# KangWelly/Assignment-for-AAE6102_GNSS-SDR

Hardware: AMD Instinct MI355X
Metric: correlator Msamples/s (acq+track), whole job (higher is better)
Workload: dtype int8 in; acquisition: f64 correlation + f64 fine search; tracking: f64

## Files before the change

### assignment-for-aae6102_gnss-sdr_amd/csrc/acq_fft.hip

```cpp
#include "gnss_internal.h"

#pragma clang fp contract(fast)

namespace gnss {

namespace {

constexpr int kRow = 2000;
constexpr int kRowPad = 2100;
constexpr int kRowThreads = 256;
constexpr int kColThreads = 256;

template <int P> struct PrimeTab;
template <> struct PrimeTab<13> {
    static constexpr double c[13] = {1.0, 0.8854560256532099, 0.5680647467311559, 0.120536680255323, -0.35460488704253545, -0.7485107481711012, -0.970941817426052, -0.9709418174260521, -0.7485107481711013, -0.3546048870425359, 0.1205366802553232, 0.5680647467311548, 0.88545602565321};
    static constexpr double s[13] = {0.0, 0.4647231720437685, 0.8229838658936564, 0.992708874098054, 0.9350162426854148, 0.6631226582407952, 0.23931566428755768, -0.23931566428755743, -0.663122658240795, -0.9350162426854147, -0.992708874098054, -0.822983865893657, -0.4647231720437684};
};
template <> struct PrimeTab<29> {
    static constexpr double c[29] = {1.0, 0.9766205557100867, 0.907575419670957, 0.7960930657056438, 0.6473862847818277, 0.46840844069979015, 0.26752833852922075, 0.05413890858541761, -0.16178199655276473, -0.37013815533991423, -0.5611870653623823, -0.7259954919231306, -0.8568571761675893, -0.9476531711828025, -0.9941379571543596, -0.9941379571543597, -0.9476531711828025, -0.8568571761675892, -0.7259954919231311, -0.5611870653623825, -0.37013815533991445, -0.16178199655276476, 0.0541389085854167, 0.2675283385292201, 0.4684084406997903, 0.6473862847818279, 0.796093065705644, 0.9075754196709569, 0.9766205557100867};
    static constexpr double s[29] = {0.0, 0.21497044021102407, 0.4198891015602646, 0.6051742151937652, 0.7621620551276365, 0.8835120444460229, 0.963549992519223, 0.9985334138511238, 0.9868265225415261, 0.9289767198167915, 0.8276889981568906, 0.6876994588534235, 0.5155538571770216, 0.3193015301359798, 0.10811901842394192, -0.10811901842394124, -0.31930153013597995, -0.5155538571770218, -0.6876994588534231, -0.8276889981568905, -0.9289767198167914, -0.9868265225415261, -0.9985334138511239, -0.9635499925192231, -0.8835120444460228, -0.7621620551276362, -0.6051742151937649, -0.41988910156026493, -0.21497044021102438};
};

template <class V> struct RealOf;
template <> struct RealOf<float2> { using T = float; };
// ... 1258 lines not shown

size_t acq_fused_sync_bytes() { return sizeof(FuseSync); }
size_t acq_fused_err_offset() { return offsetof(FuseSync, err); }
size_t acq_fused_ring_bytes(int64_t S) { return sizeof(double2) * (size_t)kFuseX * kFuseSlots * (size_t)S; }

hipError_t launch_acq_fft_correlate_fused(const double2* C, const double2* X, int64_t S, int datalen, int nbins,
                                          int nprn, int nslot, const double2* tw_row, const double2* tw_col,
                                          double2* ring, void* sync, double* corr, hipStream_t s)
{
    if (nslot < 2 || nslot > kFuseSlots) return hipErrorInvalidValue;
    const double scale = 1.0 / ((double)S * (double)S);
    int dev = 0, ncu = 0;
    hipError_t e = hipGetDevice(&dev);
    if (e == hipSuccess) e = hipDeviceGetAttribute(&ncu, hipDeviceAttributeMultiprocessorCount, dev);
    if (e == hipSuccess) e = hipMemsetAsync(sync, 0, sizeof(FuseSync), s);
    if (e != hipSuccess) return e;
    FuseSync* sy = static_cast<FuseSync*>(sync);
#define GNSS_FUSED(P_)                                                                          \
    if (S == (int64_t)P_ * kRow) {                                                              \
        int occ = 0;                                                                            \
        e = hipOccupancyMaxActiveBlocksPerMultiprocessor(&occ, inv_fused_kernel_f64<P_>, kRowThreads, 0); \
        if (e != hipSuccess) return e;                                                          \
        const int grid = ncu * std::min(occ, 2);                                                \
        if (grid < 1) return hipErrorInvalidConfiguration;                                      \
        hipLaunchKernelGGL(inv_fused_kernel_f64<P_>, dim3(grid), dim3(kRowThreads), 0, s, C, X, nbins, nprn, \
                           datalen, nbins * nprn, nslot, scale, tw_row, tw_col, ring, sy, corr); \
        return hipGetLastError();                                                               \
    }
    GNSS_FUSED(13) GNSS_FUSED(29)
#undef GNSS_FUSED
    return hipErrorInvalidValue;
}

bool fine_fft_supported(int64_t S, int L) { return acq_fft_supported(S) && L == kFineT; }

namespace {
struct FineLayout {
    int64_t M, N, tabs, slab, part;
};
FineLayout fine_layout(int64_t S, int L, int datalen)
{
    FineLayout f;
    f.M = (int64_t)L * S;
    f.N = f.M * datalen;
    f.tabs = kRow + (int64_t)kRow * datalen + (int64_t)kFineT * kRow + S + f.M / kRow + kTwIK;
    f.slab = f.N;
    f.part = (int64_t)datalen * (kRow / kFineJC);
    return f;
}
}

static size_t fine_prep_offset(const FineLayout& f, int nsv)
{
    const size_t b = sizeof(double2) * (size_t)(f.tabs + (int64_t)nsv * f.slab) + sizeof(FineBest) * (size_t)(nsv * f.part);
    return (b + 255) & ~(size_t)255;
}
size_t fine_fft_scratch_bytes(int64_t S, int L, int datalen, int nsv)
{
    const FineLayout f = fine_layout(S, L, datalen);
    if (!GNSS_FINE_PREP) return fine_prep_offset(f, nsv);
    return fine_prep_offset(f, nsv) + (size_t)nsv * f.M * (sizeof(double2) + sizeof(float));
}

hipError_t launch_fine_fft_tables(int64_t S, int L, int datalen, void* scratch, hipStream_t s)
{
    const int64_t M = (int64_t)L * S;
    double2* tw_row = static_cast<double2*>(scratch);
    double2* tabA = tw_row + kRow;
    double2* tabB = tabA + (int64_t)kRow * datalen;
    double2* tabK = tabB + (int64_t)kFineT * kRow;
    double2* tabS = tabK + S;
    const int64_t lens[5] = {kRow, (int64_t)kRow * datalen, (int64_t)kFineT * kRow, S, M / kRow};
    const int64_t divs[5] = {kRow, (int64_t)kRow * datalen, (int64_t)kFineT * kRow, M, M / kRow};
    const int64_t rows[5] = {0, kRow, kRow, kRow, 0};
    double2* tabs[5] = {tw_row, tabA, tabB, tabK, tabS};
    for (int t = 0; t < 5; t++)
        hipLaunchKernelGGL(fine_twiddle_kernel, dim3((unsigned)((lens[t] + 255) / 256)), dim3(256), 0,
                           s, tabs[t], lens[t], divs[t], rows[t]);
    hipLaunchKernelGGL(fine_twik_kernel, dim3((kTwIK + 255) / 256), dim3(256), 0, s, tw_row, tabS + M / kRow);
    return hipGetLastError();
}

hipError_t launch_fine_fft_argmax(const int8_t* iq, const double2* xs, int64_t S, int L, int datalen,
                                  const int32_t* cd, int nsv, const float* ca, double Fs, double codeFreqBasis,
                                  double codelength, int shifted, void* scratch, int64_t* kbest, hipStream_t s)
{
    if (nsv < 1 || nsv > 65535) return hipErrorInvalidValue;
    const FineLayout f = fine_layout(S, L, datalen);
    const int64_t N = f.N;
    double2* tw_row = static_cast<double2*>(scratch);
    double2* tabA = tw_row + kRow;
    double2* tabB = tabA + (int64_t)kRow * datalen;
    double2* tabK = tabB + (int64_t)kFineT * kRow;
    double2* tabS = tabK + S;
    double2* E = tw_row + f.tabs;
    FineBest* part = reinterpret_cast<FineBest*>(E + (int64_t)nsv * f.slab);
    char* prep = static_cast<char*>(scratch) + fine_prep_offset(f, nsv);
    float* ct = reinterpret_cast<float*>(prep + (size_t)nsv * f.M * sizeof(double2));
    const int nblk = kRow / kFineJC;
    auto rows = [&](auto src, auto* xt, auto kern, auto prep_kern, int tm) {
        using SrcT = decltype(src);
        if (GNSS_FINE_PREP) {
            hipLaunchKernelGGL(prep_kern, dim3((kRow + tm - 1) / tm, nsv), dim3(kRowThreads), 0, s, src, cd, S, 1 / Fs,
                               1 / codeFreqBasis, codelength, ca, xt, ct);
            src = SrcElem<SrcT>::wrap(xt);
        }
        hipLaunchKernelGGL(kern, dim3((unsigned)(f.M / kRow), datalen, nsv), dim3(kRowThreads), 0, s, src, ct, cd, S,
                           ca, 1 / Fs, 1 / codeFreqBasis, codelength, datalen, N, tw_row, tabS + f.M / kRow, tabA,
                           tabB, E);
    };
#define GNSS_FINE(P_)                                                                           \
    if (S == (int64_t)P_ * kRow) {                                                              \
        if (xs)                                                                                 \
            rows(SrcC64{xs}, reinterpret_cast<double2*>(prep), fine_rows_kernel<P_, SrcC64>,    \
                 fine_prep_kernel<P_, SrcC64>, SrcElem<SrcC64>::kTM);                           \
        else                                                                                    \
            rows(SrcIQ8{iq}, reinterpret_cast<char2*>(prep), fine_rows_kernel<P_, SrcIQ8>,      \
                 fine_prep_kernel<P_, SrcIQ8>, SrcElem<SrcIQ8>::kTM);                           \
        hipLaunchKernelGGL(fine_cols_kernel<P_>, dim3(nblk, datalen, nsv), dim3(kColThreads), 0, s, E, \
                           datalen, N, shifted, tabK, tabS, part);                                    \
        hipLaunchKernelGGL(fine_best_final_kernel, dim3(nsv), dim3(256), 0, s, part, nblk * datalen, \
                           kbest);                                                              \
        return hipGetLastError();                                                               \
    }
    GNSS_FINE(13) GNSS_FINE(29)
#undef GNSS_FINE
    return hipErrorInvalidValue;
}

}
```

### assignment-for-aae6102_gnss-sdr_amd/csrc/api_acq.cpp

```cpp
#include <cmath>
#include <cstring>
#include <vector>

#include "host.h"

using namespace gnss;
using namespace gnss::host;

namespace {
constexpr int kAcqPipeDefault = 2;
#ifndef GNSS_ACQ_FWD_SPLIT
#define GNSS_ACQ_FWD_SPLIT 1
#endif
constexpr bool kAcqFwdSplit = GNSS_ACQ_FWD_SPLIT;
constexpr int kAcqPairFront = 60;
constexpr int kFineBatch = 16;

template <class V> struct CplxReal;
template <> struct CplxReal<float2> { using T = float; };
template <> struct CplxReal<double2> { using T = double; };

template <class V>
int acq_search(gnss_ctx* ctx, const int8_t* blk, const double2* xa, int64_t S, int dl, int nb, int np,
               const gnss_signal* sg, const gnss_acq* acq, const float* ca, typename CplxReal<V>::T* corr,
// ... 300 lines not shown
        return fail(ctx, GNSS_EDEVICE, "fused correlator: a pipeline wait timed out (grid not resident)");
    ctx->timing.acq_hypothesis_samples = (int64_t)np * nb * dl * S;

    std::vector<int> acq_idx;
    for (int i = 0; i < np; i++) {
        if (diag) {
            int k = diag->n++;
            diag->prn[k] = prns[i];
            diag->SNR[k] = ph[i].snr;
            diag->fbin[k] = ph[i].fbin + 1;
            diag->codePhase[k] = ph[i].cp + 1;
            diag->peak[k] = ph[i].peak;
            diag->peak2[k] = ph[i].peak2;
        }
        if (ph[i].snr >= 12) {
            int k = out->n++;
            out->sv[k] = prns[i];
            out->SNR[k] = ph[i].snr;
            out->Doppler[k] = acq->freqMin + acq->freqStep * (double)ph[i].fbin;
            out->codedelay[k] = ph[i].cp;
            acq_idx.push_back(i);
        }
    }
    if (out->n == 0) {
        HIP_TRY(hipEventRecord(e_all.b, ctx->stream));
        HIP_TRY(hipEventSynchronize(e_all.b));
        ctx->timing.acq_ms = e_all.ms();
        ctx->timing.acq_corr_ms = ctx->timing.acq_ms;
        return fail(ctx, GNSS_ENODATA, "No satellites acquired");
    }

    if (flen < off + S * bps * (L + 1)) return fail(ctx, GNSS_EIO, "IF record too short for fine search");
    const int fshift = dtyp == 2 ? 1 : 2;
    const int na = out->n;
    const int64_t N = (int64_t)L * S * dl;
    if (N % 2) return fail(ctx, GNSS_EINDEX, "odd fftlength: MATLAB indexes past the end (:116)");
    std::vector<float> caf((size_t)na * 1023);
    std::vector<int32_t> cdh((size_t)na);
    for (int k = 0; k < na; k++) {
        generate_ca(out->sv[k], &caf[(size_t)k * 1023]);
        cdh[k] = out->codedelay[k];
    }
    DevBuf fca, fcd, fx, kb;
    HIP_TRY(fca.alloc(ctx, "acq.fca", caf.size() * sizeof(float)));
    HIP_TRY(fcd.alloc(ctx, "acq.fcd", cdh.size() * sizeof(int32_t)));
    HIP_TRY(kb.alloc(ctx, "acq.kb", sizeof(int64_t) * (size_t)na));
    HIP_TRY(hipMemcpyAsync(fca.p, caf.data(), caf.size() * sizeof(float), hipMemcpyHostToDevice, ctx->stream));
    HIP_TRY(hipMemcpyAsync(fcd.p, cdh.data(), cdh.size() * sizeof(int32_t), hipMemcpyHostToDevice, ctx->stream));
    const bool own_fine = fine_fft_supported(S, L) && !ctx->opt[GNSS_OPT_FINE_ROCFFT];
    Events e_fine;
    if (own_fine) {
        const int fb = std::min(na, kFineBatch);
        HIP_TRY(fx.alloc(ctx, "acq.fx", fine_fft_scratch_bytes(S, L, dl, fb)));
        HIP_TRY(hipEventRecord(e_fine.a, ctx->stream));
        HIP_TRY(launch_fine_fft_tables(S, L, dl, fx.p, ctx->stream));
        for (int k0 = 0; k0 < na; k0 += fb) {
            const int nk = std::min(fb, na - k0);
            HIP_TRY(launch_fine_fft_argmax(blk, xf, S, L, dl, fcd.as<int32_t>() + k0, nk,
                                           fca.as<float>() + (size_t)k0 * 1023, sg->Fs, sg->codeFreqBasis,
                                           sg->codelength, fshift, fx.p, kb.as<int64_t>() + k0, ctx->stream));
        }
    } else {
        HIP_TRY(fx.alloc(ctx, "acq.fx", sizeof(double2) * (size_t)na * N));
        rocfft_plan pl;
        if ((st = get_plan(ctx, N, na, 1, 0, &pl))) return st;
        HIP_TRY(hipEventRecord(e_fine.a, ctx->stream));
        HIP_TRY(launch_fine_build(blk, xf, S, L, fcd.as<int32_t>(), fca.as<float>(), na, sg->Fs, sg->codeFreqBasis,
                                  sg->codelength, N, fx.as<double2>(), ctx->stream));
        if ((st = run_fft(ctx, fx.p, N, na, 1, 0))) return st;
        DevBuf fscr;
        HIP_TRY(fscr.alloc(ctx, "acq.fscr", acq_scratch_bytes(1, na)));
        HIP_TRY(launch_fine_argmax(fx.as<double2>(), na, N, fshift, fscr.p, kb.as<int64_t>(), ctx->stream));
    }
    HIP_TRY(hipEventRecord(e_fine.b, ctx->stream));
    HIP_TRY(hipEventRecord(e_all.b, ctx->stream));
    std::vector<int64_t> kh((size_t)na);
    HIP_TRY(hipMemcpyAsync(kh.data(), kb.p, sizeof(int64_t) * (size_t)na, hipMemcpyDeviceToHost, ctx->stream));
    HIP_TRY(hipStreamSynchronize(ctx->stream));
    for (int k = 0; k < na; k++) {
        const double K = (double)kh[k];
        out->fineFreq[k] = (file->dataType == 2) ? (-K * (sg->Fs / (double)N) + sg->Fs / 2) : (K * (sg->Fs / (double)N));
    }
    {
        float f = 0;
        (void)hipEventElapsedTime(&f, e_all.a, e_corr.b);
        ctx->timing.acq_corr_ms = f;
    }
    ctx->timing.acq_fine_ms = e_fine.ms();
    ctx->timing.acq_ms = e_all.ms() + (iq8 ? 0.0 : e_conv.ms());
    return GNSS_OK;
}

}
```

### assignment-for-aae6102_gnss-sdr_amd/csrc/gnss_internal.h

```cpp
#pragma once

#include <hip/hip_runtime.h>
#include <stdint.h>

#include "../../include/gnss_mi355x.h"

#define GNSS_HD __host__ __device__ __forceinline__

namespace gnss {

struct Colon {
    double a, d, c;
    int64_t n;
};

GNSS_HD Colon colon_make(double a, double d, double b)
{
    Colon r{a, d, b, -1};
    if (!(a - a == 0) || !(d - d == 0) || !(b - b == 0)) return r;
    if (d == 0 || (a < b && d < 0) || (b < a && d > 0)) return r;
    double tol = 2.0 * 2.220446049250313e-16 * fmax(fabs(a), fabs(b));
    double sig = d > 0 ? 1.0 : -1.0;
    double n;
    if (a == floor(a) && d == 1) {
// ... 362 lines not shown
    int32_t cp;
    double snr;
    double peak2;
};

hipError_t launch_acq_wipe(const int8_t* iq, const double2* xs, int64_t S, int datalen, int nbins, double IF,
                           double freqMin, double freqStep, double Fs, float2* out, hipStream_t s);
hipError_t launch_acq_code(const float* ca, const int32_t* prn_slot, int nprn, int64_t S,
                           double codeFreqBasis, double Fs, float2* out, hipStream_t s);
hipError_t launch_acq_mul(const float2* code_spec, const float2* sig_spec, int nprn, int nsig,
                          int64_t S, float2* out, hipStream_t s);
hipError_t launch_acq_power(const float2* y, int nprn, int nbins, int datalen, int64_t S,
                            int first_ms, float* corr, hipStream_t s);
hipError_t launch_acq_wipe(const int8_t* iq, const double2* xs, int64_t S, int datalen, int nbins, double IF,
                           double freqMin, double freqStep, double Fs, double2* out, hipStream_t s);
hipError_t launch_acq_code(const float* ca, const int32_t* prn_slot, int nprn, int64_t S,
                           double codeFreqBasis, double Fs, double2* out, hipStream_t s);
hipError_t launch_acq_mul(const double2* code_spec, const double2* sig_spec, int nprn, int nsig,
                          int64_t S, double2* out, hipStream_t s);
hipError_t launch_acq_power(const double2* y, int nprn, int nbins, int datalen, int64_t S,
                            int first_ms, double* corr, hipStream_t s);
hipError_t launch_acq_peak(const float* corr, int nprn, int nbins, int64_t S, int cshift,
                           int perm, AcqPeak* out, void* scratch, hipStream_t s);
hipError_t launch_acq_peak(const double* corr, int nprn, int nbins, int64_t S, int cshift,
                           int perm, AcqPeak* out, void* scratch, hipStream_t s);

bool acq_fft_supported(int64_t S);
template <class V>
hipError_t launch_acq_fft_forward(const int8_t* iq, const double2* xs, int64_t S, int datalen, int nbins, double IF,
                                  double freqMin, double freqStep, double Fs, const float* ca,
                                  int nprn, double codeFreqBasis, const V* tw_row,
                                  const V* tw_col, V* B, V* X, hipStream_t s, int bin0 = 0, int nbc = -1,
                                  bool codes = true);
constexpr int kAcqCols = 1, kAcqRows = 2;
hipError_t launch_acq_fft_correlate(const float2* C, const float2* X, int64_t S, int datalen,
                                    int nbins, int nprn, int first_pair, int npair,
                                    const float2* tw_row, const float2* tw_col, float2* A,
                                    float* corr, hipStream_t s, int parts = kAcqCols | kAcqRows);
hipError_t launch_acq_fft_correlate(const double2* C, const double2* X, int64_t S, int datalen,
                                    int nbins, int nprn, int first_pair, int npair,
                                    const double2* tw_row, const double2* tw_col, double2* A,
                                    double* corr, hipStream_t s, int parts = kAcqCols | kAcqRows);
hipError_t launch_acq_fft_pair(const double2* C, const double2* X, int64_t S, int datalen, int nbins, int nprn,
                               int cols_first, int cols_n, double2* Acols, int rows_first, int rows_n,
                               const double2* Arows, const double2* tw_row, const double2* tw_col, double* corr,
                               int front, hipStream_t s);
size_t acq_fused_sync_bytes();
size_t acq_fused_err_offset();
size_t acq_fused_ring_bytes(int64_t S);
hipError_t launch_acq_fft_correlate_fused(const double2* C, const double2* X, int64_t S, int datalen, int nbins,
                                          int nprn, int nslot, const double2* tw_row, const double2* tw_col,
                                          double2* ring, void* sync, double* corr, hipStream_t s);
bool fine_fft_supported(int64_t S, int L);
size_t fine_fft_scratch_bytes(int64_t S, int L, int datalen, int nsv);
hipError_t launch_fine_fft_tables(int64_t S, int L, int datalen, void* scratch, hipStream_t s);
hipError_t launch_fine_fft_argmax(const int8_t* iq, const double2* xs, int64_t S, int L, int datalen,
                                  const int32_t* cd, int nsv, const float* ca, double Fs, double codeFreqBasis,
                                  double codelength, int shifted, void* scratch, int64_t* kbest, hipStream_t s);
hipError_t launch_fine_build(const int8_t* iq, const double2* xs, int64_t S, int L, const int32_t* codedelay,
                             const float* ca, int nsv, double Fs, double codeFreqBasis,
                             double codelength, int64_t N, double2* out, hipStream_t s);
hipError_t launch_fine_argmax(const double2* F, int nsv, int64_t N, int shifted, void* scratch,
                              int64_t* kbest, hipStream_t s);

size_t acq_scratch_bytes(int nprn, int nsv);

hipError_t launch_stage_cpx(const int8_t* src, int prec, int type, int64_t nsamp, double2* out,
                            unsigned long long* sums, hipStream_t s);
hipError_t launch_real8_to_iq8(const int8_t* src, int64_t n, int8_t* dst, hipStream_t s);
size_t prefix16_scratch_bytes(int64_t ngroups);
hipError_t launch_prefix16(const short* src, int64_t ngroups, long long* pref_i, long long* pref_q,
                           void* scratch, size_t scratch_bytes, hipStream_t s);

struct SrcIQ8 {
    const int8_t* p;
    __device__ __forceinline__ double2 at(int64_t n) const
    {
        const char2 r = *reinterpret_cast<const char2*>(p + 2 * n);
        return make_double2((double)r.x, (double)r.y);
    }
};
struct SrcC64 {
    const double2* p;
    __device__ __forceinline__ double2 at(int64_t n) const { return p[n]; }
};


GNSS_HD double cn0_moment(const double* Z, double T)
{
    double mean = 0;
    for (int k = 0; k < 20; k++) mean += Z[k];
    mean = mean / 20;
    double var = 0;
    for (int k = 0; k < 20; k++) var += (Z[k] - mean) * (Z[k] - mean);
    var = var / 19;
    const double m2v = mean * mean - var;
    const double scale = 1 / T;
    if (m2v >= 0) {
        const double NA2 = sqrt(m2v);
        const double varIQ = 0.5 * (mean - NA2);
        return fabs(10 * log10(scale * NA2 / (2 * varIQ)));
    }
    const double y = sqrt(-m2v);
    const double nr = 0, ni = scale * y;
    const double dr = 2 * (0.5 * mean), di = 2 * (0.5 * -y);
    const double den = dr * dr + di * di;
    const double zr = (nr * dr + ni * di) / den, zi = (ni * dr - nr * di) / den;
    const double lr = 10 * (log(hypot(zr, zi)) / log(10.0));
    const double li = 10 * (atan2(zi, zr) / log(10.0));
    return hypot(lr, li);
}
// ... 227 lines not shown
```

### assignment-for-aae6102_gnss-sdr_amd/csrc/host.h

```cpp
#pragma once

#include <hip/hip_runtime.h>
#include <rocfft/rocfft.h>

#include <algorithm>
#include <cstdint>
#include <cstdlib>
#include <map>
#include <string>
#include <thread>
#include <tuple>
#include <utility>
#include <vector>

#include "gnss_internal.h"
#include "group.h"

struct gnss_ctx {
    int device = 0;
    hipStream_t stream = nullptr;
    hipStream_t stream2 = nullptr;
    hipEvent_t ev_cols[2] = {}, ev_rows[2] = {};
    std::string err;
    gnss_timing timing{};
    int profiling = 0;
    std::map<std::tuple<size_t, size_t, int, int>, rocfft_plan> plans;
    void* fft_work = nullptr;
    size_t fft_work_size = 0;
    std::map<std::string, std::pair<void*, size_t>> pool;
    std::map<std::string, std::pair<void*, size_t>> pinned;
    int64_t acq_tw_S = 0;
    int acq_tw_dbl = -1;
    int acq_fp64 = 1;
    uint64_t window = 0;
    int64_t opt[GNSS_OPT_COUNT] = {};
    int lane_path = 0;
    std::vector<gnss_ctx*> members;
    bool member = false;
    int fail_chan = -1;
    gnss::group::ResidentCache<void*> resident;
};

namespace gnss {
struct AcfDev;
struct AcfExtPlan;
namespace host {

inline const char* probe_env(const char* name)
{
    return GNSS_PROBE_BUILD ? getenv(name) : nullptr;
}

constexpr int kVtSpan = 2000;

int fail(gnss_ctx* ctx, int code, const char* fmt, ...) __attribute__((format(printf, 3, 4)));

#define HIP_TRY(expr)                                                                         \
    do {                                                                                       \
        hipError_t e_ = (expr);                                                                \
        if (e_ != hipSuccess)                                                                  \
            return ::gnss::host::fail(ctx, GNSS_EDEVICE, "%s:%d %s: %s", __FILE__, __LINE__,   \
                                      #expr, hipGetErrorString(e_));                           \
    } while (0)

template <class T>
T* pinned_buffer(gnss_ctx* ctx, const char* key, size_t count, unsigned flags = hipHostMallocDefault)
{
    auto& e = ctx->pinned[key];
    const size_t want = std::max<size_t>(count * sizeof(T), 16);
    if (e.second < want) {
        if (e.first) (void)hipHostFree(e.first);
        e = {nullptr, 0};
        if (hipHostMalloc(&e.first, want, flags) != hipSuccess) return nullptr;
        e.second = want;
    }
    return static_cast<T*>(e.first);
}

struct DevBuf {
    void* p = nullptr;
    size_t n = 0;
    bool pooled = false;
    DevBuf() = default;
    DevBuf(const DevBuf&) = delete;
    DevBuf& operator=(const DevBuf&) = delete;
// ... 106 lines not shown
```

### assignment-for-aae6102_gnss-sdr_amd/csrc/track.hip

```cpp
#include "gnss_internal.h"

#include <cstddef>
#include <type_traits>
#include <utility>

namespace gnss {

namespace {

constexpr int kStampRow = 8 + 3 * kMaxBpc;

__device__ __forceinline__ unsigned long long* stamp_row(const TrkBuffers& b)
{
    const unsigned long long cnt = __hip_atomic_load(b.stamps + (size_t)kStampSlots * kStampRow,
                                                     __ATOMIC_RELAXED, __HIP_MEMORY_SCOPE_AGENT);
    return b.stamps + (cnt % kStampSlots) * kStampRow;
}

__device__ __forceinline__ void stamp_max(unsigned long long* row, int k, unsigned long long v)
{
    row[k] = v;
}

__device__ __forceinline__ int uni(int v) { return __builtin_amdgcn_readfirstlane(v); }
// ... 445 lines not shown
    if (Index >= c.sv1) cols = (int64_t)((uint32_t)(Index - c.sv1) / (uint32_t)p.nsv) + 1;
    return cols > nstep ? nstep : cols;
}

__device__ __forceinline__ void write_record_i(const TrkParams& p, const TrkBuffers& b, int ch, const TrkChan& c,
                             const StepOut& o, const LoopUpd& u, const double* s,
                             const int64_t* pre = nullptr, int part = 3)
{
    const double P_i = s[2 * p.iP], P_q = s[2 * p.iP + 1];
    const int64_t slot = c.slot;
    g_dbl* r = (g_dbl*)(b.rec + ((int64_t)ch * p.rec_cap + slot) * GNSS_NFIELDS);
    if (part & 1) {
        const int64_t col = c.nstep;
        g_i64* dvpre = (g_i64*)(b.dvpre + (int64_t)ch * (p.rec_cap + 1));
        const int64_t dvsum = (pre ? pre[0] : dvpre[col]) + o.delayValue;
        dvpre[col + 1] = dvsum;
        const int64_t nstep = col + 1;
        const int64_t cols = record_cols(p, c, o.phaseC);
        const double codedelay =
            (double)c.codedelay0 + (double)(cols == nstep ? dvsum : (pre ? pre[1] : dvpre[cols]));
        if (slot < p.rec_cap) {
            r[GNSS_F_P_i] = P_i;                     r[GNSS_F_P_q] = P_q;
            r[GNSS_F_E_i] = s[2 * p.iE];             r[GNSS_F_E_q] = s[2 * p.iE + 1];
            r[GNSS_F_L_i] = s[2 * p.iL];             r[GNSS_F_L_q] = s[2 * p.iL + 1];
            r[GNSS_F_codedelay] = codedelay;
        }
    }
    if (part & 2) {
        const int64_t pos = c.pos + p.bps * o.n;
        const double absS = (double)pos;
        const double m = fmod_pos(absS / p.dataBytesPerSample, p.Fs * p.ms);
        if (slot < p.rec_cap) {
            r[GNSS_F_PLLdiscri] = u.PLLdiscri;       r[GNSS_F_DLLdiscri] = u.DLLdiscri;
            r[GNSS_F_remChip] = o.remChip;
            r[GNSS_F_codeFreq] = u.codeFreq;         r[GNSS_F_carrierFreq] = u.carrierFreq;
            r[GNSS_F_remPhase] = o.remPhase;         r[GNSS_F_remSample] = p.conv ? m : o.remSample;
            r[GNSS_F_numSample] = (double)o.n;       r[GNSS_F_delayValue] = (double)o.delayValue;
            r[GNSS_F_absoluteSample] = absS;         r[GNSS_F_codedelay2] = m;
        }
        if (!o.phaseC && slot < b.n1) ((g_dbl*)b.p_i_1ms)[(int64_t)ch * b.n1 + slot] = P_i;
    }
}
__device__ __noinline__ void write_record(const TrkParams& p, const TrkBuffers& b, int ch, const TrkChan& c, const StepOut& o, const LoopUpd& u, const double* s)
{
    write_record_i(p, b, ch, c, o, u, s);
}


__device__ __noinline__ double cn0_estimate(const double (&Z)[20], double T)
{
    return cn0_moment(Z, T);
}

__device__ __forceinline__ void write_state_i(const TrkParams& p, const TrkBuffers& b, int ch, TrkChan* g,
                            const TrkChan& c, const StepOut& o, const LoopUpd& u, const double* s,
                            bool io = true)
{
    const double P_i = s[2 * p.iP], P_q = s[2 * p.iP + 1];
    int index_int = c.index_int + 1;
    int snrIndex = c.snrIndex;
    const double zk = P_i * P_i + P_q * P_q;
    for (int k = 0; k < 20; k++) g->Zk[k] = k == index_int - 1 ? zk : c.Zk[k];
    if (index_int % 20 == 0 && io) {
        double Z[20];
#pragma unroll
        for (int k = 0; k < 20; k++) Z[k] = k == index_int - 1 ? zk : c.Zk[k];
        const double cn = cn0_estimate(Z, 1 * p.ms * o.pdi);
        double* cn0 = o.phaseC ? b.cn0_10 : b.cn0_1;
        if (snrIndex <= p.cn0_cap) cn0[(int64_t)ch * p.cn0_cap + snrIndex - 1] = cn;
        index_int = 0;
        snrIndex += 1;
    } else if (index_int % 20 == 0) {
        index_int = 0;
        snrIndex += 1;
    }
    g->remChip = o.remChip;
    g->remPhase = o.remPhase;
    g->remSample = o.remSample;
    g->carrier_outputLast = u.carrier_output;
    g->PLLdiscriLast = u.PLLdiscri;
    g->code_outputLast = u.code_output;
    g->DLLdiscriLast = u.DLLdiscri;
    g->codeFreq = u.codeFreq;
    g->carrierFreq = u.carrierFreq;
    g->numSample = o.n;
    g->pos = c.pos + p.bps * o.n;
    g->Index = c.Index + (o.phaseC ? 10 : 1);
    g->nstep = c.nstep + 1;
    g->slot = c.slot + 1;
    g->index_int = index_int;
    g->snrIndex = snrIndex;
}
__device__ __noinline__ void write_state(const TrkParams& p, const TrkBuffers& b, int ch, TrkChan* g, const TrkChan& c, const StepOut& o, const LoopUpd& u, const double* s, bool io)
{
    write_state_i(p, b, ch, g, c, o, u, s, io);
}

__device__ __forceinline__ void update_state_inplace(const TrkParams& p, const TrkBuffers& b, int ch,
                                                     TrkChan& c, const StepOut& o, const LoopUpd& u,
                                                     const double* s, bool io)
{
    const double P_i = s[2 * p.iP], P_q = s[2 * p.iP + 1];
    int index_int = c.index_int + 1;
    int snrIndex = c.snrIndex;
    c.Zk[index_int - 1] = P_i * P_i + P_q * P_q;
    if (index_int % 20 == 0) {
        if (io) {
            double Z[20];
#pragma unroll
            for (int k = 0; k < 20; k++) Z[k] = c.Zk[k];
            const double cn = cn0_estimate(Z, 1 * p.ms * o.pdi);
            g_dbl* cn0 = (g_dbl*)(o.phaseC ? b.cn0_10 : b.cn0_1);
            if (snrIndex <= p.cn0_cap) cn0[(int64_t)ch * p.cn0_cap + snrIndex - 1] = cn;
        }
        index_int = 0;
        snrIndex += 1;
    }
    const int64_t pos = c.pos, Index = c.Index, nstep = c.nstep, slot = c.slot;
    c.remChip = o.remChip;
    c.remPhase = o.remPhase;
    c.remSample = o.remSample;
    c.carrier_outputLast = u.carrier_output;
    c.PLLdiscriLast = u.PLLdiscri;
    c.code_outputLast = u.code_output;
    c.DLLdiscriLast = u.DLLdiscri;
    c.codeFreq = u.codeFreq;
    c.carrierFreq = u.carrierFreq;
    c.numSample = o.n;
    c.pos = pos + p.bps * o.n;
    c.Index = Index + (o.phaseC ? 10 : 1);
    c.nstep = nstep + 1;
    c.slot = slot + 1;
    c.index_int = index_int;
    c.snrIndex = snrIndex;
}


}

__device__ __forceinline__ double2 ld_rcs(const StepDesc* d, int m) { return d->rcs[m]; }
__device__ __forceinline__ double2 ld_rcs(g_desc* d, int m)
{
    typedef __attribute__((address_space(1))) const double g_cdbl;
    g_cdbl* q = (g_cdbl*)&d->rcs[m];
    return make_double2(q[0], q[1]);
}

template <int SUB> struct RegRaw {
    const int4 (&r)[SUB];
    __device__ __forceinline__ int4 get(int j) const { return r[j]; }
};
struct LdsRaw {
    const int4* p;
    __device__ __forceinline__ int4 get(int j) const { return p[j * kTrkThreads]; }
};
typedef __attribute__((address_space(3))) const char lds_cchar;
typedef __attribute__((address_space(3))) const double lds_cdbl;
typedef double dbl2v __attribute__((ext_vector_type(2)));
typedef __attribute__((address_space(3))) const dbl2v lds_cdbl2;

template <class F, int... I>
__device__ __forceinline__ void static_for_seq(F&& f, std::integer_sequence<int, I...>)
{
    (f(std::integral_constant<int, I>{}), ...);
// ... 1010 lines not shown
        while ((st = __hip_atomic_load((g_u32*)state, __ATOMIC_RELAXED, __HIP_MEMORY_SCOPE_AGENT)) == 0) {
            if (wall_clock64() - t0 > 2000000ull) atomicCAS(state, 0u, 2u);
            __builtin_amdgcn_s_sleep(2);
        }
        if (st == 2) atomicCAS(w, 0u, 2u);
        s_go = st == 1;
    }
    __syncthreads();
    return s_go != 0;
}

template <int SUB>
__device__ __forceinline__ void prefetch_raw(const int8_t* iq, int64_t g0, int64_t gmax, int4* s_raw,
                                             int tid)
{
    const int wbase = tid & ~63;
#pragma unroll
    for (int j = 0; j < SUB; j++) {
        int64_t gj = g0 + j;
        gj = gj < gmax ? gj : gmax;
        __builtin_amdgcn_global_load_lds((__attribute__((address_space(1))) void*)(iq + 16 * gj),
                                         (__attribute__((address_space(3))) void*)(s_raw + j * kTrkThreads + wbase),
                                         16, 0, 0);
    }
}

#ifndef GNSS_DEFER
#define GNSS_DEFER 0
#endif
#ifndef GNSS_WPE_TAPS
#define GNSS_WPE_TAPS 2
#endif
template <int NT, int SUB, bool DIVIDE, bool VB = false, bool REGC = false>
__global__ __launch_bounds__(kTrkThreads) __attribute__((amdgpu_waves_per_eu(NT > 3 ? GNSS_WPE_TAPS : 3, NT > 3 ? GNSS_WPE_TAPS : 3))) void track_run_kernel(const TrkParams* __restrict__ pp,
                                                               const TrkBuffers* __restrict__ bp, int bpc,
                                                               int vpb, int nsteps, unsigned tag0)
{
    const TrkParams& p = *pp;
    const TailK tk = tail_k(p);
    const TrkBuffers& b = *bp;
    constexpr int M = 8 * SUB;
    constexpr int NV = 2 * NT;
    constexpr int T = kTrkThreads;
    static_assert(M <= kLaneMax, "lane span exceeds the rotation table");
    const int vpb_ = VB ? vpb : 1;
    const int pbpc = (bpc + vpb_ - 1) / vpb_;
    const bool xl = GNSS_XCD_LOCAL == 1 && !VB && p.nch == 8;
    const bool cul = GNSS_XCD_LOCAL == 2 && !VB && p.nch == 8 && pbpc == 96;
    const int ch = xl ? (int)(blockIdx.x & 7) : cul ? (int)((blockIdx.x & 255) >> 5) : (int)(blockIdx.x / pbpc);
    const int pblk = xl ? (int)(blockIdx.x >> 3)
                    : cul ? (int)((blockIdx.x & 31) * 3 + (blockIdx.x >> 8)) : (int)(blockIdx.x - ch * pbpc);
    const int blk = pblk * vpb_;
    const int nvb = VB ? (bpc - blk < vpb_ ? bpc - blk : vpb_) : 1;
    const int tid = threadIdx.x, lane = tid & 63, wv = tid >> 6;
    const bool io = pblk == 0;

    constexpr int kSlot = REGC ? 0 : 8 * T * 2;
    constexpr int kRed = red_words<run_red_taps<NT>()>();
    constexpr int kPart = run_bpc_cap(NT) * NV;
    constexpr bool kDefer = GNSS_DEFER && NT > 3;
    constexpr bool kWave1 = GNSS_DEFER == 2 && kDefer && !VB;
    static_assert(!kWave1 || GNSS_RED == 0, "GNSS_DEFER 2 needs GNSS_RED 0");
    constexpr int kPwD = run_bpc_cap(NT) * 8 + 2 * NT;
    constexpr int kStage = 2 * (NT - 1) * T;
    constexpr int kMemW = kWave1 ? kPwD + kStage + 2 * NT * 32 : 0;
    constexpr int kMem1 = kSlot > kRed ? kSlot : kRed;
    constexpr int kMem0 = kMem1 > kMemW ? kMem1 : kMemW;
    constexpr int kMem = kMem0 > kPart + 16 * NV ? kMem0 : kPart + 16 * NV;
    __shared__ __attribute__((aligned(16))) double s_mem[kMem];
    __shared__ __attribute__((aligned(16))) int4 s_raw[SUB * T];
    __shared__ __attribute__((aligned(16))) StepDesc s_d[2];
    __shared__ __attribute__((aligned(16))) TrkChan s_c;
    __shared__ StepOut s_o;
    __shared__ LoopUpd s_u;
    __shared__ double s_fin[NV];
    __shared__ double s_taps[GNSS_MAX_TAPS], s_post[GNSS_MAX_TAPS];
    __shared__ double2 s_zero;

    if (!census(b.run_err, tid)) return;
    g_chan* cp = (g_chan*)(b.chan + ch);
    if (cp->status != GNSS_OK) return;
    const int64_t n1_target = cp->n1_target;
    const int8_t* iq = b.iq - p.buf_base;
    const int64_t gmax = (p.buf_base + p.buf_len) / 16 - 1;
    const unsigned cabits = ca_bits_ext(lane < 32 ? ((g_cu32*)b.ca_bits)[ch * 32 + lane] : 0u, lane);
    const __amdgpu_buffer_rsrc_t pg = __builtin_amdgcn_make_buffer_rsrc(
        b.pgran + (int64_t)ch * 2 * gran_per_chan(NT), (short)0, gran_per_chan(NT) * 16, kBufRsrcWord3);
    constexpr int kChanWords = (int)(sizeof(TrkChan) / 8);

    constexpr int CL = chan_lanes<NV>();
    constexpr int HT = run_red_taps<NT>();
    struct DeferCfg {
        unsigned selA, selB;
        int NA, nBv, hb, own_lo, own_n, bneg;
        int64_t bslot;
        int vmap[kDefer ? NV : 1];
    };
    __shared__ DeferCfg s_df;
    typedef __attribute__((address_space(3))) volatile const int lds_vint;
    typedef __attribute__((address_space(3))) volatile const long long lds_vi64;
    auto dfi = [&](const int& f) { return uni((int)*(lds_vint*)&f); };
    auto NA_ = [&]() { return kDefer ? dfi(s_df.NA) : NV; };
    auto own_n_ = [&]() { return kDefer ? dfi(s_df.own_n) : 0; };
    const bool dob = kDefer && b.taps_rec != nullptr;
    if constexpr (kDefer) {
        if (tid == 0) {
            unsigned selA = 0, selB = 0;
// ... 112 lines not shown
        double a = 0.0;
        if (lane < nbv * 4) {
            const double* r = r2 + (lane >> 2) * 32 + (lane & 3) * 8;
            a = r[0];
#pragma unroll
            for (int k = 1; k < 8; k++) a += r[k];
            a += dpp_f64<0xB1>(a);
            a += dpp_f64<0x4E>(a);
            if ((lane & 3) == 0)
                publish16(pg, gran_region_b(NT) + (step & 3) * gran_slot_b(NT) + (lane >> 2) * bpc + blk, a,
                          tag0 + step + 1);
        }
    };
    auto flush = [&]() {
        if (wv == 1) {
            unsigned long long* fr = kProbe && (GNSS_FLUSH_PROBE & 2) && b.stamps && ch == 0 && io && lane == 0
                                         ? b.stamps + (size_t)(s_now % kStampSlots) * kStampRow : nullptr;
            if (fr) fr[2000] = wall_clock64();
            if (lane == 0 && !(GNSS_FLUSH_PROBE & 1)) {
                if (dio) {
                    if (!pre_ok) {
                        asm volatile("s_waitcnt vmcnt(0)" ::: "memory");
                        const g_i64* dvp = (const g_i64*)(b.dvpre + (int64_t)ch * (p.rec_cap + 1));
                        const int64_t cols = record_cols(p, s_c, s_o.phaseC);
                        pre[1] = cols < s_c.nstep + 1 ? dvp[cols] : 0;
                    }
                    pre[0] = dvrun;
                    write_record_i(p, b, ch, s_c, s_o, s_u, s_fin, pre, duty_b == duty_a ? 3 : 1);
                    dvrun += s_o.delayValue;
                }
                else if (pblk == duty_b) write_record_i(p, b, ch, s_c, s_o, s_u, s_fin, nullptr, 2);
            }
            if (fr) {
                fr[2001] = wall_clock64();
                write_record_i(p, b, ch, s_c, s_o, s_u, s_fin, pre, 3);
                fr[2002] = wall_clock64();
            }
            if (pblk == duty_b && b.taps_rec && lane < NA_() && s_c.slot < p.rec_cap) {
                const int v = kDefer ? s_df.vmap[lane] : lane;
                ((g_dbl*)b.taps_rec)[((int64_t)ch * p.rec_cap + s_c.slot) * NV + v] = s_fin[v];
            }
            if (kDefer && lane == 0) {
                s_df.bslot = s_c.slot;
                s_df.bneg = s_o.phaseC;
            }
            if (lane == 0) update_state_inplace(p, b, ch, s_c, s_o, s_u, s_fin, pblk == duty_c);
        }
        pend = false;
        pre_ok = false;
    };
    const unsigned long long t_start = kProbe ? wall_clock64() : 0ull;
    for (int s = 0; s < nsteps; s++) {
        s_now = s;
        const StepDesc& D = s_d[cur];
        const int bad = D.bad ? D.bad : D.bad_tap;
        const bool stop = !D.phaseC && D.Index + 1 > n1_target;
        if (bad || stop || D.d * M >= 1.0 || (GNSS_QCAP && NT > kQcapMax && D.d > tk.qcap_dmax)) {
            const bool had = pend;
            if (pend) flush();
            if (had) defer_final(s - 1);
            if (io && tid == 64) desc_rem(tk, &s_d[cur]);
            __syncthreads();
            if (io) {
                if (tid == 0 && !stop) s_c.status = bad ? bad : GNSS_EINDEX;
                __syncthreads();
                if (tid < kChanWords)
                    reinterpret_cast<uint64_t*>(b.chan + ch)[tid] = reinterpret_cast<const uint64_t*>(&s_c)[tid];
                for (int e = tid; e < kDescWords; e += T)
                    reinterpret_cast<unsigned*>(b.desc + ch)[e] = reinterpret_cast<const unsigned*>(&D)[e];
            }
            return;
        }
        const int64_t A = uni(D.A), n = uni(D.n);
        unsigned long long* srow = kProbe && b.stamps && ch == 0 && (io || pblk == pbpc - 1)
                                       ? b.stamps + (size_t)(s % kStampSlots) * kStampRow + (io ? 0 : 5) : nullptr;
        if (srow && tid == 0) srow[0] = wall_clock64();
        unsigned long long* brow = kProbe && b.stamps && ch == 0 ? b.stamps + (size_t)(s % kStampSlots) * kStampRow : nullptr;
        if (brow && tid == 0) brow[40 + blk] = wall_clock64();

        for (int jv = 0; jv < nvb; jv++) {
            const int vb = blk + jv;
            switch ((kProbe && (p.probe & 64)) ? ch % 3 : (kProbe && (p.probe & 128)) ? 0 : (s + ch) % 3) {
            case 0: __builtin_amdgcn_s_setprio(0); break;
            case 1: __builtin_amdgcn_s_setprio(1); break;
            default: __builtin_amdgcn_s_setprio(2); break;
            }
            {
                const int64_t g0 = uni(D.g_first) + ((int64_t)vb * T + tid) * SUB;
                asm volatile("s_waitcnt vmcnt(0)" ::: "memory");
                double oI[NT], oQ[NT];
                lane_correlate<NT, SUB, DIVIDE, true, 0, REGC>(p, &D, LdsRaw{s_raw + tid}, 8 * g0 - A, cabits,
                                                      reinterpret_cast<double2*>(s_mem) + tid, &s_zero, oI, oQ,
                                                      s_post);
                __syncthreads();
                if (pend && dio && wv == 1 && lane == 0 && jv == 0) {
                    asm volatile("s_waitcnt vmcnt(0)" ::: "memory");
                    const g_i64* dvp = (const g_i64*)(b.dvpre + (int64_t)ch * (p.rec_cap + 1));
                    const int64_t cols = record_cols(p, s_c, s_o.phaseC);
                    pre[1] = cols < s_c.nstep + 1 ? dvp[cols] : 0;
                    pre_ok = true;
                }
                if (VB && jv + 1 < nvb)
                    prefetch_raw<SUB>(iq, uni(D.g_first) + ((int64_t)(vb + 1) * T + tid) * SUB, gmax, s_raw, tid);
                __builtin_amdgcn_s_setprio(3);
                if (srow && tid == 0) srow[1] = wall_clock64();
                if (brow && tid == 0) brow[40 + 256 + vb] = wall_clock64();
                if constexpr (!kDefer) {
                    const double bsum = block_partial<NT, HT>(s_mem, oI, oQ, tid);
                    if (tid < NV * 4 && (tid & 3) == 0)
                        publish16(pg, ((s & 1) * kMaxBpcRun + vb) * NV + (tid >> 2), bsum, tag0 + s + 1);
                } else {
                    const double ba = block_pass<NT, HT>(s_mem, oI, oQ, tid, (unsigned)dfi(*(const int*)&s_df.selA));
                    const int NA = NA_();
                    if (tid < NA * 4 && (tid & 3) == 0)
                        publish16(pg, ((s & 1) * kMaxBpcRun + vb) * NA + (tid >> 2), ba, tag0 + s + 1);
                    if (kWave1 && dob) {
                        double* stg = s_mem + kPwD;
                        const unsigned sb = (unsigned)dfi(*(const int*)&s_df.selB);
#pragma unroll
                        for (int s2 = 0; s2 < NT; s2++)
                            if ((sb >> s2) & 1u) {
                                const int r = __builtin_popcount(sb & ((1u << s2) - 1u));
                                stg[(2 * r) * T + tid] = oI[s2];
                                stg[(2 * r + 1) * T + tid] = oQ[s2];
                            }
                        lds_barrier();
                    } else if (dob) {
                        const int hb = dfi(s_df.hb), nB = dfi(s_df.nBv) / 2;
                        for (int ps = 1; (ps - 1) * hb < nB; ps++) {
                            const unsigned sel = sel_pass(ps);
                            const double bb = block_pass<NT, HT>(s_mem, oI, oQ, tid, sel);
                            if (tid < 2 * __builtin_popcount(sel) * 4 && (tid & 3) == 0)
                                publish16(pg, gran_region_b(NT) + (s & 3) * gran_slot_b(NT) +
                                                  (2 * (ps - 1) * hb + (tid >> 2)) * bpc + vb,
                                          bb, tag0 + s + 1);
                        }
                    }
                }
                if (srow && tid == 0) srow[2] = wall_clock64();
                if (kProbe && b.stamps && ch == 0 && tid == 0) {
                    unsigned long long* r = b.stamps + (size_t)(s % kStampSlots) * kStampRow;
                    atomicMax(r + 23, wall_clock64());
                    atomicMax(r + 24, ~wall_clock64());
                }
            }
// ... 372 lines not shown
```

Baseline: 400,900.

## Cache fine-FFT twiddle tables across calls and tweak tracking register pressure

Moves the fine-search FFT twiddle tables into their own buffer. The context remembers the (S, L, datalen) they were built for, so table generation is skipped when those match a previous call. Separately, the tracking kernel gets a noinline C/N0 helper that reads Zk directly instead of copying it to a local array. It also re-derives lane and wave ids from an opaque copy of the thread id each step, to cut register pressure or live ranges. The table reuse depends on the DevBuf allocation persisting with the same contents across calls, which is not visible here.

```diff
diff --git a/assignment-for-aae6102_gnss-sdr_amd/csrc/acq_fft.hip b/assignment-for-aae6102_gnss-sdr_amd/csrc/acq_fft.hip
--- a/assignment-for-aae6102_gnss-sdr_amd/csrc/acq_fft.hip
+++ b/assignment-for-aae6102_gnss-sdr_amd/csrc/acq_fft.hip
@@ -1334,8 +1334,12 @@
 
 static size_t fine_prep_offset(const FineLayout& f, int nsv)
 {
-    const size_t b = sizeof(double2) * (size_t)(f.tabs + (int64_t)nsv * f.slab) + sizeof(FineBest) * (size_t)(nsv * f.part);
+    const size_t b = sizeof(double2) * (size_t)((int64_t)nsv * f.slab) + sizeof(FineBest) * (size_t)(nsv * f.part);
     return (b + 255) & ~(size_t)255;
+}
+size_t fine_fft_table_bytes(int64_t S, int L, int datalen)
+{
+    return sizeof(double2) * (size_t)fine_layout(S, L, datalen).tabs;
 }
 size_t fine_fft_scratch_bytes(int64_t S, int L, int datalen, int nsv)
 {
@@ -1344,10 +1348,10 @@
     return fine_prep_offset(f, nsv) + (size_t)nsv * f.M * (sizeof(double2) + sizeof(float));
 }
 
-hipError_t launch_fine_fft_tables(int64_t S, int L, int datalen, void* scratch, hipStream_t s)
+hipError_t launch_fine_fft_tables(int64_t S, int L, int datalen, void* tables, hipStream_t s)
 {
     const int64_t M = (int64_t)L * S;
-    double2* tw_row = static_cast<double2*>(scratch);
+    double2* tw_row = static_cast<double2*>(tables);
     double2* tabA = tw_row + kRow;
     double2* tabB = tabA + (int64_t)kRow * datalen;
     double2* tabK = tabB + (int64_t)kFineT * kRow;
@@ -1365,17 +1369,18 @@
 
 hipError_t launch_fine_fft_argmax(const int8_t* iq, const double2* xs, int64_t S, int L, int datalen,
                                   const int32_t* cd, int nsv, const float* ca, double Fs, double codeFreqBasis,
-                                  double codelength, int shifted, void* scratch, int64_t* kbest, hipStream_t s)
+                                  double codelength, int shifted, const void* tables, void* scratch,
+                                  int64_t* kbest, hipStream_t s)
 {
     if (nsv < 1 || nsv > 65535) return hipErrorInvalidValue;
     const FineLayout f = fine_layout(S, L, datalen);
     const int64_t N = f.N;
-    double2* tw_row = static_cast<double2*>(scratch);
-    double2* tabA = tw_row + kRow;
-    double2* tabB = tabA + (int64_t)kRow * datalen;
-    double2* tabK = tabB + (int64_t)kFineT * kRow;
-    double2* tabS = tabK + S;
-    double2* E = tw_row + f.tabs;
+    const double2* tw_row = static_cast<const double2*>(tables);
+    const double2* tabA = tw_row + kRow;
+    const double2* tabB = tabA + (int64_t)kRow * datalen;
+    const double2* tabK = tabB + (int64_t)kFineT * kRow;
+    const double2* tabS = tabK + S;
+    double2* E = static_cast<double2*>(scratch);
     FineBest* part = reinterpret_cast<FineBest*>(E + (int64_t)nsv * f.slab);
     char* prep = static_cast<char*>(scratch) + fine_prep_offset(f, nsv);
     float* ct = reinterpret_cast<float*>(prep + (size_t)nsv * f.M * sizeof(double2));
diff --git a/assignment-for-aae6102_gnss-sdr_amd/csrc/api_acq.cpp b/assignment-for-aae6102_gnss-sdr_amd/csrc/api_acq.cpp
--- a/assignment-for-aae6102_gnss-sdr_amd/csrc/api_acq.cpp
+++ b/assignment-for-aae6102_gnss-sdr_amd/csrc/api_acq.cpp
@@ -376,13 +376,23 @@
     if (own_fine) {
         const int fb = std::min(na, kFineBatch);
         HIP_TRY(fx.alloc(ctx, "acq.fx", fine_fft_scratch_bytes(S, L, dl, fb)));
+        DevBuf ftw;
+        const bool have_ftw = ctx->fine_tw_S == S && ctx->fine_tw_L == L && ctx->fine_tw_dl == dl;
+        HIP_TRY(ftw.alloc(ctx, "acq.fine_tw", fine_fft_table_bytes(S, L, dl)));
         HIP_TRY(hipEventRecord(e_fine.a, ctx->stream));
-        HIP_TRY(launch_fine_fft_tables(S, L, dl, fx.p, ctx->stream));
+        if (!have_ftw) {
+            ctx->fine_tw_S = 0;
+            HIP_TRY(launch_fine_fft_tables(S, L, dl, ftw.p, ctx->stream));
+            ctx->fine_tw_S = S;
+            ctx->fine_tw_L = L;
+            ctx->fine_tw_dl = dl;
+        }
         for (int k0 = 0; k0 < na; k0 += fb) {
             const int nk = std::min(fb, na - k0);
             HIP_TRY(launch_fine_fft_argmax(blk, xf, S, L, dl, fcd.as<int32_t>() + k0, nk,
                                            fca.as<float>() + (size_t)k0 * 1023, sg->Fs, sg->codeFreqBasis,
-                                           sg->codelength, fshift, fx.p, kb.as<int64_t>() + k0, ctx->stream));
+                                           sg->codelength, fshift, ftw.p, fx.p, kb.as<int64_t>() + k0,
+                                           ctx->stream));
         }
     } else {
         HIP_TRY(fx.alloc(ctx, "acq.fx", sizeof(double2) * (size_t)na * N));
diff --git a/assignment-for-aae6102_gnss-sdr_amd/csrc/gnss_internal.h b/assignment-for-aae6102_gnss-sdr_amd/csrc/gnss_internal.h
--- a/assignment-for-aae6102_gnss-sdr_amd/csrc/gnss_internal.h
+++ b/assignment-for-aae6102_gnss-sdr_amd/csrc/gnss_internal.h
@@ -438,11 +438,13 @@
                                           int nprn, int nslot, const double2* tw_row, const double2* tw_col,
                                           double2* ring, void* sync, double* corr, hipStream_t s);
 bool fine_fft_supported(int64_t S, int L);
+size_t fine_fft_table_bytes(int64_t S, int L, int datalen);
 size_t fine_fft_scratch_bytes(int64_t S, int L, int datalen, int nsv);
-hipError_t launch_fine_fft_tables(int64_t S, int L, int datalen, void* scratch, hipStream_t s);
+hipError_t launch_fine_fft_tables(int64_t S, int L, int datalen, void* tables, hipStream_t s);
 hipError_t launch_fine_fft_argmax(const int8_t* iq, const double2* xs, int64_t S, int L, int datalen,
                                   const int32_t* cd, int nsv, const float* ca, double Fs, double codeFreqBasis,
-                                  double codelength, int shifted, void* scratch, int64_t* kbest, hipStream_t s);
+                                  double codelength, int shifted, const void* tables, void* scratch,
+                                  int64_t* kbest, hipStream_t s);
 hipError_t launch_fine_build(const int8_t* iq, const double2* xs, int64_t S, int L, const int32_t* codedelay,
                              const float* ca, int nsv, double Fs, double codeFreqBasis,
                              double codelength, int64_t N, double2* out, hipStream_t s);
diff --git a/assignment-for-aae6102_gnss-sdr_amd/csrc/host.h b/assignment-for-aae6102_gnss-sdr_amd/csrc/host.h
--- a/assignment-for-aae6102_gnss-sdr_amd/csrc/host.h
+++ b/assignment-for-aae6102_gnss-sdr_amd/csrc/host.h
@@ -31,6 +31,8 @@
     std::map<std::string, std::pair<void*, size_t>> pinned;
     int64_t acq_tw_S = 0;
     int acq_tw_dbl = -1;
+    int64_t fine_tw_S = 0;
+    int fine_tw_L = 0, fine_tw_dl = 0;
     int acq_fp64 = 1;
     uint64_t window = 0;
     int64_t opt[GNSS_OPT_COUNT] = {};
diff --git a/assignment-for-aae6102_gnss-sdr_amd/csrc/track.hip b/assignment-for-aae6102_gnss-sdr_amd/csrc/track.hip
--- a/assignment-for-aae6102_gnss-sdr_amd/csrc/track.hip
+++ b/assignment-for-aae6102_gnss-sdr_amd/csrc/track.hip
@@ -521,6 +521,11 @@
     return cn0_moment(Z, T);
 }
 
+__device__ __noinline__ double cn0_estimate_at(const double* Z, double T)
+{
+    return cn0_moment(Z, T);
+}
+
 __device__ __forceinline__ void write_state_i(const TrkParams& p, const TrkBuffers& b, int ch, TrkChan* g,
                             const TrkChan& c, const StepOut& o, const LoopUpd& u, const double* s,
                             bool io = true)
@@ -575,10 +580,7 @@
     c.Zk[index_int - 1] = P_i * P_i + P_q * P_q;
     if (index_int % 20 == 0) {
         if (io) {
-            double Z[20];
-#pragma unroll
-            for (int k = 0; k < 20; k++) Z[k] = c.Zk[k];
-            const double cn = cn0_estimate(Z, 1 * p.ms * o.pdi);
+            const double cn = cn0_estimate_at(c.Zk, 1 * p.ms * o.pdi);
             g_dbl* cn0 = (g_dbl*)(o.phaseC ? b.cn0_10 : b.cn0_1);
             if (snrIndex <= p.cn0_cap) cn0[(int64_t)ch * p.cn0_cap + snrIndex - 1] = cn;
         }
@@ -1695,7 +1697,8 @@
                     : cul ? (int)((blockIdx.x & 31) * 3 + (blockIdx.x >> 8)) : (int)(blockIdx.x - ch * pbpc);
     const int blk = pblk * vpb_;
     const int nvb = VB ? (bpc - blk < vpb_ ? bpc - blk : vpb_) : 1;
-    const int tid = threadIdx.x, lane = tid & 63, wv = tid >> 6;
+    const int tid0 = threadIdx.x;
+    int tid = tid0, lane = tid & 63, wv = tid >> 6;
     const bool io = pblk == 0;
 
     constexpr int kSlot = REGC ? 0 : 8 * T * 2;
@@ -1914,6 +1917,9 @@
     const unsigned long long t_start = kProbe ? wall_clock64() : 0ull;
     for (int s = 0; s < nsteps; s++) {
         s_now = s;
+        asm volatile("" : "+v"(tid));
+        lane = tid & 63;
+        wv = tid >> 6;
         const StepDesc& D = s_d[cur];
         const int bad = D.bad ? D.bad : D.bad_tap;
         const bool stop = !D.phaseC && D.Index + 1 > n1_target;
@@ -1948,11 +1954,11 @@
             default: __builtin_amdgcn_s_setprio(2); break;
             }
             {
-                const int64_t g0 = uni(D.g_first) + ((int64_t)vb * T + tid) * SUB;
+                const int64_t g0 = uni(D.g_first) + ((int64_t)vb * T + tid0) * SUB;
                 asm volatile("s_waitcnt vmcnt(0)" ::: "memory");
                 double oI[NT], oQ[NT];
-                lane_correlate<NT, SUB, DIVIDE, true, 0, REGC>(p, &D, LdsRaw{s_raw + tid}, 8 * g0 - A, cabits,
-                                                      reinterpret_cast<double2*>(s_mem) + tid, &s_zero, oI, oQ,
+                lane_correlate<NT, SUB, DIVIDE, true, 0, REGC>(p, &D, LdsRaw{s_raw + tid0}, 8 * g0 - A, cabits,
+                                                      reinterpret_cast<double2*>(s_mem) + tid0, &s_zero, oI, oQ,
                                                       s_post);
                 __syncthreads();
                 if (pend && dio && wv == 1 && lane == 0 && jv == 0) {
```

Result: no change. 402,200 (median of 6 runs) (+0.3%).
